# facebookresearch/seamless_communication

Measured on AMD Instinct MI355X. Metric: S2ST utterances/sec (and real-time factor), seamlessM4T_v2_large, 10 s audio, higher is better.
Workload: dtype f32 activations x f16 weights, f32 accumulate

## Files before the change

### seamless_communication_amd/csrc/common.cpp

```cpp
#include "common.h"
#include <cstdlib>
#include <cstring>

namespace sc {

static thread_local char g_err[1024] = "";

void set_error(const char* fmt, ...) {
    va_list ap;
    va_start(ap, fmt);
    vsnprintf(g_err, sizeof(g_err), fmt, ap);
    va_end(ap);
}

const char* get_error() { return g_err; }

namespace knob {
namespace {
struct Knob {
    const char* name;
    int kind;
    const char* what;
};
const Knob knob_table[] = {
    {"SC_DEBUG_NUMERICS", 0, "honour the switches that change results"},
    {"SC_DEBUG_FILL", 0, "fill fresh scratch blocks with NaN (tests)"},
    {"SC_SPLIT_MODE", 1, "1: Conformer products on the hi fp16 plane only (precision study)"},
    {"SC_DECODER_GEN1", 1, "decoder step on the first-generation kernels"},
    {"SC_DECODER_GEN2", 1, "decoder step on the second-generation chain"},
    {"SC_VOC_SPLIT", 1, "vocoder ResBlock products on both fp16 planes of their activations again (bit 0 wide stages, bit 2 narrow stages); default: hi plane only"},
    {"SC_GEMM_GENERAL", 0, "general GEMM kernel instead of the fast path"}, {"SC_GEMM_PF2", 0, "GEMM prefetch depth"},
    {"SC_GEMM_GROUP_M", 0, "GEMM workgroup order"}, {"SC_GEMM_TILE", 0, "GEMM tile override"},
    {"SC_PS_TILE", 0, "DMA GEMM: largest tile"}, {"SC_PS_MIN256", 0, "DMA GEMM: tiles needed for 256 x 256"},
    {"SC_PS_MIN128", 0, "DMA GEMM: tiles needed for 128 x 128"},
    {"SC_PRESPLIT", 0, "0: Conformer operands split on the fly"}, {"SC_ENC_FUSE", 0, "0: separate Conformer element-wise launches"},
    {"SC_D3_RG_SMALL", 0, "decoder step: rows per row group, N = 1024 products"}, {"SC_D3_RG_FFN", 0, "decoder step: rows per row group, FFN-in"},
    {"SC_G3_STATIONARY", 0, "row-group products of wide steps: 0 one workgroup per row group, n = workgroup budget of the weight-stationary launch"},
    {"SC_G3_TILES", 0, "0: FFN-out of wide steps on the weight-stationary row-group walk instead of tile-owning waves"},
    {"SC_G3_TOUCH", 0, "weight-stationary products: bit 0 cooperative L2 touch of the activations, bit 1 K slices per XCD (FFN-out); default 3"},
    {"SC_D3_FFN_IN", 0, "decoder step: FFN-in workgroup shape"}, {"SC_D3_FFN_OUT", 0, "decoder step: FFN-out workgroup shape"},
    {"SC_T2U_GROUPS", 0, "NAR T2U: length buckets"}, {"SC_T2U_PACKED", 0, "0: NAR decoder on padded buckets"},
    {"SC_VOC_PS", 0, "0: vocoder wide stages on the register-staged convolution"}, {"SC_VOC_MRF", 0, "0: narrow vocoder stages as nine pair launches"},
    {"SC_VOC_GROUPS", 0, "vocoder: length buckets"}, {"SC_VOC_GROUP_OVERHEAD", 0, "vocoder: bucket planning overhead rows"},
    {"SC_VOC_STREAMS", 0, "vocoder: side chains"},
    {"SC_VOC_PACKED", 0, "0: ragged vocoder batches in length buckets on side chains instead of the packed pass"},
    {"SC_VOC_PACK_ROWS", 0, "vocoder: unit rows per packed group"},
    {"SC_ENGINE_RG_SMALL", 0, "decode engine: rows per row group, N = 1024 products"},
    {"SC_BEAM_COMPACT", 2, "0: beam search keeps finished utterances' slots"},
    {"SC_GREEDY_COMPACT", 2, "0: greedy generation keeps finished rows in their slots"}, {"SC_GREEDY_POLL", 2, "steps between looks at the finished flags"},
    {"SC_T2U_ENC_PACKED", 2, "0: T2U encoder over the padded rows on the fp32-operand GEMM"},
    {"SC_ENC_GLU_EPI", 2, "0: Conformer conv module writes both GLU halves and gates them in the depthwise kernel"},
};
constexpr int N_KNOBS = sizeof(knob_table) / sizeof(knob_table[0]);
struct State {
    bool set[N_KNOBS];
    int val[N_KNOBS];
    bool numerics = false;
};
const State& state() {
    static const State st = [] {
        State s{};
        const char* dn = getenv("SC_DEBUG_NUMERICS");
        s.numerics = dn && atoi(dn) != 0;
        for (int i = 0; i < N_KNOBS; ++i) {
            const char* e = getenv(knob_table[i].name);
            s.set[i] = e != nullptr && (knob_table[i].kind != 1 || s.numerics);
            s.val[i] = e ? atoi(e) : 0;
        }
        return s;
    }();
    return st;
}
int lookup(const char* name) {
    for (int i = 0; i < N_KNOBS; ++i)
        if (strcmp(knob_table[i].name, name) == 0) return i;
    return -1;
}
int find(const char* name) {
    const int i = lookup(name);
    if (i >= 0) return i;
    fprintf(stderr, "libseamless_hip: switch %s is not in the knob table (common.cpp)\n", name);
    abort();
}
}

bool known(const char* name) { return name && lookup(name) >= 0; }

int value(const char* name, int dflt) {
    const int i = find(name);
    return state().set[i] ? state().val[i] : dflt;
}
bool is_set(const char* name) { return state().set[find(name)]; }
int live(const char* name, int dflt) {
    (void)find(name);
    const char* e = getenv(name);
    return e ? atoi(e) : dflt;
}
void report_once() {
    static const bool done = [] {
        const State& s = state();
        for (int i = 0; i < N_KNOBS; ++i) {
            const char* e = getenv(knob_table[i].name);
            if (!e || knob_table[i].kind == 2) continue;
            if (knob_table[i].kind == 1 && !s.numerics)
                fprintf(stderr, "libseamless_hip: %s=%s IGNORED - it changes results (%s); set SC_DEBUG_NUMERICS=1 to honour it\n", knob_table[i].name, e,
                        knob_table[i].what);
            else
                fprintf(stderr, "libseamless_hip: %s=%s (%s)%s\n", knob_table[i].name, e, knob_table[i].what, knob_table[i].kind == 1 ? " - RESULTS CHANGE" : "");
        }
        return true;
    }();
    (void)done;
}
}

}
```

### seamless_communication_amd/csrc/k_norm.hip

```cpp
#include <vector>

#include "device_util.h"

namespace sc {

__device__ __forceinline__ float act_f(float v, int a) {
    if (a == ACT_RELU) return relu_keep_nan(v);
    if (a == ACT_SILU) return v / (1.f + expf(-v));
    if (a == ACT_GELU) return gelu_erf(v);
    return v;
}

template <int MAXV>
__global__ __launch_bounds__(256) void layernorm_kernel(const float* __restrict__ x, int64_t ldx,
                                                        const float* __restrict__ gamma,
                                                        const float* __restrict__ beta,
                                                        float* __restrict__ y, int64_t ldy, int rows,
                                                        int C, int act, const int* __restrict__ lens,
                                                        int t_per_batch, __half* __restrict__ yh = nullptr,
                                                        __half* __restrict__ yl = nullptr, int64_t ldh = 0) {
    const int lane = threadIdx.x & 63;
    const int row = blockIdx.x * 4 + (threadIdx.x >> 6);
    if (row >= rows) return;
    const int nv = C >> 2;
    const float4* xr = reinterpret_cast<const float4*>(x + (int64_t)row * ldx);
    float4* yr = reinterpret_cast<float4*>(y + (int64_t)row * ldy);
    half4_t* yhr = reinterpret_cast<half4_t*>(yh + (yh ? (int64_t)row * ldh : 0));
    half4_t* ylr = reinterpret_cast<half4_t*>(yl + (yl ? (int64_t)row * ldh : 0));
    const bool both = y != nullptr && yh != nullptr;
    bool masked = false;
    if (lens) {
        const int n = row / t_per_batch;
        const int t = row - n * t_per_batch;
        if (t >= lens[n]) {
            for (int i = lane; i < nv; i += 64) {
                if (yh) {
                    yhr[i] = half4_t{0, 0, 0, 0};
                    ylr[i] = half4_t{0, 0, 0, 0};
                } else {
                    yr[i] = make_float4(0.f, 0.f, 0.f, 0.f);
                }
            }
            if (!both) return;
            masked = true;
        }
    }
    float4 v[MAXV];
    float s = 0.f;
#pragma unroll
    for (int i = 0; i < MAXV; ++i) {
        const int idx = lane + 64 * i;
        v[i] = idx < nv ? xr[idx] : make_float4(0.f, 0.f, 0.f, 0.f);
        s += (v[i].x + v[i].y) + (v[i].z + v[i].w);
    }
    const float mean = wave_sum(s) / (float)C;
    float q = 0.f;
#pragma unroll
    for (int i = 0; i < MAXV; ++i) {
        const int idx = lane + 64 * i;
        if (idx < nv) {
            const float a = v[i].x - mean, b = v[i].y - mean, c = v[i].z - mean, d = v[i].w - mean;
            q += (a * a + b * b) + (c * c + d * d);
        }
    }
    const float var = wave_sum(q) / (float)C;
    const float rstd = 1.0f / sqrtf(var + 1e-5f);
    const float4* g4 = reinterpret_cast<const float4*>(gamma);
    const float4* b4 = reinterpret_cast<const float4*>(beta);
#pragma unroll
    for (int i = 0; i < MAXV; ++i) {
        const int idx = lane + 64 * i;
        if (idx < nv) {
            const float4 g = g4[idx], b = b4[idx];
            float4 o;
            o.x = act_f((v[i].x - mean) * rstd * g.x + b.x, act);
            o.y = act_f((v[i].y - mean) * rstd * g.y + b.y, act);
            o.z = act_f((v[i].z - mean) * rstd * g.z + b.z, act);
            o.w = act_f((v[i].w - mean) * rstd * g.w + b.w, act);
            if (yh && !masked) {
                const f32x4_t of = {o.x, o.y, o.z, o.w};
                const half4_t hi = __builtin_convertvector(of, half4_t);
                const f32x4_t back = __builtin_convertvector(hi, f32x4_t);
                yhr[idx] = hi;
                ylr[idx] = __builtin_convertvector(of - back, half4_t);
            }
            if (!yh || both) yr[idx] = o;
        }
    }
}

__global__ __launch_bounds__(256) void layernorm2_kernel(const float* __restrict__ x, int64_t ldx, const float* __restrict__ ga,
                                                         const float* __restrict__ ba, float* __restrict__ y, int64_t ldy,
                                                         const float* __restrict__ gb2, const float* __restrict__ bb2,
                                                         __half* __restrict__ yh, __half* __restrict__ yl, int64_t ldh, int rows, int C) {
    const int lane = threadIdx.x & 63;
    const int row = blockIdx.x * 4 + (threadIdx.x >> 6);
    if (row >= rows) return;
    const int nv = C >> 2;
    const float4* xr = reinterpret_cast<const float4*>(x + (int64_t)row * ldx);
    float4* yr = reinterpret_cast<float4*>(y + (int64_t)row * ldy);
    half4_t* yhr = reinterpret_cast<half4_t*>(yh + (int64_t)row * ldh);
    half4_t* ylr = reinterpret_cast<half4_t*>(yl + (int64_t)row * ldh);
    float4 v[4];
    float s = 0.f;
#pragma unroll
    for (int i = 0; i < 4; ++i) {
        const int idx = lane + 64 * i;
        v[i] = idx < nv ? xr[idx] : make_float4(0.f, 0.f, 0.f, 0.f);
        s += (v[i].x + v[i].y) + (v[i].z + v[i].w);
    }
    float mean = wave_sum(s) / (float)C;
    float q = 0.f;
#pragma unroll
    for (int i = 0; i < 4; ++i) {
        const int idx = lane + 64 * i;
        if (idx < nv) {
            const float a = v[i].x - mean, b = v[i].y - mean, c = v[i].z - mean, d = v[i].w - mean;
            q += (a * a + b * b) + (c * c + d * d);
        }
    }
    float rstd = 1.0f / sqrtf(wave_sum(q) / (float)C + 1e-5f);
    s = 0.f;
#pragma unroll
    for (int i = 0; i < 4; ++i) {
        const int idx = lane + 64 * i;
        if (idx < nv) {
            const float4 g = reinterpret_cast<const float4*>(ga)[idx], b = reinterpret_cast<const float4*>(ba)[idx];
            v[i].x = (v[i].x - mean) * rstd * g.x + b.x;
            v[i].y = (v[i].y - mean) * rstd * g.y + b.y;
            v[i].z = (v[i].z - mean) * rstd * g.z + b.z;
            v[i].w = (v[i].w - mean) * rstd * g.w + b.w;
            yr[idx] = v[i];
        }
        s += (v[i].x + v[i].y) + (v[i].z + v[i].w);
    }
    mean = wave_sum(s) / (float)C;
    q = 0.f;
#pragma unroll
    for (int i = 0; i < 4; ++i) {
        const int idx = lane + 64 * i;
        if (idx < nv) {
            const float a = v[i].x - mean, b = v[i].y - mean, c = v[i].z - mean, d = v[i].w - mean;
            q += (a * a + b * b) + (c * c + d * d);
        }
    }
    rstd = 1.0f / sqrtf(wave_sum(q) / (float)C + 1e-5f);
#pragma unroll
    for (int i = 0; i < 4; ++i) {
        const int idx = lane + 64 * i;
        if (idx < nv) {
            const float4 g = reinterpret_cast<const float4*>(gb2)[idx], b = reinterpret_cast<const float4*>(bb2)[idx];
            const f32x4_t of = {(v[i].x - mean) * rstd * g.x + b.x, (v[i].y - mean) * rstd * g.y + b.y, (v[i].z - mean) * rstd * g.z + b.z,
                             (v[i].w - mean) * rstd * g.w + b.w};
            const half4_t hi = __builtin_convertvector(of, half4_t);
            const f32x4_t back = __builtin_convertvector(hi, f32x4_t);
            yhr[idx] = hi;
            ylr[idx] = __builtin_convertvector(of - back, half4_t);
        }
    }
}

void launch_layernorm2_split(const float* x, int64_t ldx, const float* ga, const float* ba, float* y, int64_t ldy, const float* gb2,
                             const float* bb2, __half* yh, __half* yl, int64_t ldh, int rows, int C, hipStream_t s) {
    SC_CHECK(C % 4 == 0 && C <= 1024 && ldx % 4 == 0 && ldy % 4 == 0 && ldh % 4 == 0 && y && yh && yl, "layernorm2_split: C=%d", C);
    if (rows <= 0) return;
    hipLaunchKernelGGL(layernorm2_kernel, dim3(cdiv(rows, 4)), dim3(256), 0, s, x, ldx, ga, ba, y, ldy, gb2, bb2, yh, yl, ldh, rows, C);
    SC_LAUNCH_CHECK();
}

void launch_layernorm_split(const float* x, int64_t ldx, const float* gamma, const float* beta, __half* yh, __half* yl,
                            int64_t ldh, int rows, int C, int act, const int* lens, int t_per_batch, hipStream_t s) {
    SC_CHECK(C % 4 == 0 && ldx % 4 == 0 && ldh % 4 == 0 && C <= 4096 && yh && yl, "layernorm_split: C=%d ldx=%lld ldh=%lld", C,
             (long long)ldx, (long long)ldh);
    if (rows <= 0) return;
    dim3 grid(cdiv(rows, 4));
    float* none = nullptr;
    if (C <= 256) hipLaunchKernelGGL((layernorm_kernel<1>), grid, dim3(256), 0, s, x, ldx, gamma, beta, none, (int64_t)0, rows, C, act, lens, t_per_batch, yh, yl, ldh);
    else if (C <= 1024) hipLaunchKernelGGL((layernorm_kernel<4>), grid, dim3(256), 0, s, x, ldx, gamma, beta, none, (int64_t)0, rows, C, act, lens, t_per_batch, yh, yl, ldh);
    else hipLaunchKernelGGL((layernorm_kernel<16>), grid, dim3(256), 0, s, x, ldx, gamma, beta, none, (int64_t)0, rows, C, act, lens, t_per_batch, yh, yl, ldh);
    SC_LAUNCH_CHECK();
}

void launch_layernorm_both(const float* x, int64_t ldx, const float* gamma, const float* beta, float* y, int64_t ldy, __half* yh,
                           __half* yl, int64_t ldh, int rows, int C, int act, const int* lens, int t_per_batch, hipStream_t s) {
    SC_CHECK(C % 4 == 0 && ldx % 4 == 0 && ldy % 4 == 0 && ldh % 4 == 0 && C <= 4096 && y && yh && yl, "layernorm_both: C=%d", C);
    if (rows <= 0) return;
    dim3 grid(cdiv(rows, 4));
    if (C <= 256) hipLaunchKernelGGL((layernorm_kernel<1>), grid, dim3(256), 0, s, x, ldx, gamma, beta, y, ldy, rows, C, act, lens, t_per_batch, yh, yl, ldh);
    else if (C <= 1024) hipLaunchKernelGGL((layernorm_kernel<4>), grid, dim3(256), 0, s, x, ldx, gamma, beta, y, ldy, rows, C, act, lens, t_per_batch, yh, yl, ldh);
    else hipLaunchKernelGGL((layernorm_kernel<16>), grid, dim3(256), 0, s, x, ldx, gamma, beta, y, ldy, rows, C, act, lens, t_per_batch, yh, yl, ldh);
    SC_LAUNCH_CHECK();
}

void launch_layernorm(const float* x, int64_t ldx, const float* gamma, const float* beta, float* y,
                      int64_t ldy, int rows, int C, int act, const int* lens, int t_per_batch,
                      hipStream_t s) {
    SC_CHECK(C % 4 == 0 && ldx % 4 == 0 && ldy % 4 == 0, "layernorm: C=%d ldx=%lld ldy=%lld must be multiples of 4", C,
             (long long)ldx, (long long)ldy);
    SC_CHECK(C <= 4096, "layernorm: C=%d > 4096 unsupported", C);
    if (rows <= 0) return;
    dim3 grid(cdiv(rows, 4));
    if (C <= 256) {
        hipLaunchKernelGGL((layernorm_kernel<1>), grid, dim3(256), 0, s, x, ldx, gamma, beta, y, ldy, rows, C, act, lens, t_per_batch, (__half*)nullptr, (__half*)nullptr, (int64_t)0);
    } else if (C <= 1024) {
        hipLaunchKernelGGL((layernorm_kernel<4>), grid, dim3(256), 0, s, x, ldx, gamma, beta, y, ldy, rows, C, act, lens, t_per_batch, (__half*)nullptr, (__half*)nullptr, (int64_t)0);
    } else {
        hipLaunchKernelGGL((layernorm_kernel<16>), grid, dim3(256), 0, s, x, ldx, gamma, beta, y, ldy, rows, C, act, lens, t_per_batch, (__half*)nullptr, (__half*)nullptr, (int64_t)0);
    }
    SC_LAUNCH_CHECK();
}

__global__ __launch_bounds__(256) void glu_kernel(const float* __restrict__ x, int64_t ldx,
                                                  float* __restrict__ y, int64_t ldy, int rows, int C) {
    const int cv = C >> 2;
    const int64_t total = (int64_t)rows * cv;
    for (int64_t i = (int64_t)blockIdx.x * blockDim.x + threadIdx.x; i < total;
         i += (int64_t)gridDim.x * blockDim.x) {
        const int r = (int)(i / cv);
        const int c = (int)(i - (int64_t)r * cv);
        const float4 a = *reinterpret_cast<const float4*>(x + (int64_t)r * ldx + c * 4);
        const float4 g = *reinterpret_cast<const float4*>(x + (int64_t)r * ldx + C + c * 4);
        float4 o;
        o.x = a.x / (1.f + expf(-g.x));
        o.y = a.y / (1.f + expf(-g.y));
        o.z = a.z / (1.f + expf(-g.z));
        o.w = a.w / (1.f + expf(-g.w));
        *reinterpret_cast<float4*>(y + (int64_t)r * ldy + c * 4) = o;
    }
}

void launch_glu(const float* x, int64_t ldx, float* y, int64_t ldy, int rows, int C, hipStream_t s) {
    SC_CHECK(C % 4 == 0 && ldx % 4 == 0 && ldy % 4 == 0, "glu: alignment");
    if (rows <= 0) return;
    const int64_t total = (int64_t)rows * (C / 4);
    const int blocks = (int)std::min<int64_t>(cdiv64(total, 256), 4096);
    hipLaunchKernelGGL(glu_kernel, dim3(blocks), dim3(256), 0, s, x, ldx, y, ldy, rows, C);
    SC_LAUNCH_CHECK();
}

template <int K, int TT>
__global__ __launch_bounds__(256) void glu_dwconv_kernel(const float* __restrict__ x, int64_t ldx,
                                                         const float* __restrict__ w,
                                                         float* __restrict__ y, int64_t ldy, int T,
                                                         int C, const int* __restrict__ lens, int left,
                                                         const float* __restrict__ bn_scale,
                                                         const float* __restrict__ bn_shift) {
    const int c = blockIdx.x * 256 + threadIdx.x;
    const int t0 = blockIdx.y * TT;
    const int n = blockIdx.z;
    if (c >= C) return;
    const int len = lens ? min(lens[n], T) : T;
    float wr[K];
#pragma unroll
    for (int j = 0; j < K; ++j) wr[j] = w[c * K + j];
    float g[TT + K - 1];
#pragma unroll
    for (int i = 0; i < TT + K - 1; ++i) {
        const int t = t0 - left + i;
        float v = 0.f;
        if (t >= 0 && t < len) {
            const float* xr = x + ((int64_t)n * T + t) * ldx;
            const float a = xr[c];
            const float b = xr[C + c];
            v = a / (1.f + expf(-b));
        }
        g[i] = v;
    }
#pragma unroll
    for (int tt = 0; tt < TT; ++tt) {
        const int t = t0 + tt;
        if (t < T) {
            float acc = 0.f;
#pragma unroll
            for (int j = 0; j < K; ++j) acc = fmaf(wr[j], g[tt + j], acc);
            if (bn_scale) {
                acc = fmaf(acc, bn_scale[c], bn_shift[c]);
                acc = acc / (1.f + expf(-acc));
            }
            y[((int64_t)n * T + t) * ldy + c] = acc;
        }
    }
}

__global__ __launch_bounds__(256) void glu_dwconv_generic_kernel(const float* __restrict__ x, int64_t ldx,
                                                                 const float* __restrict__ w,
                                                                 float* __restrict__ y, int64_t ldy,
                                                                 int T, int C, int K,
                                                                 const int* __restrict__ lens, int left,
                                                                 const float* __restrict__ bn_scale,
                                                                 const float* __restrict__ bn_shift) {
    const int c = blockIdx.x * 256 + threadIdx.x;
    const int t = blockIdx.y;
    const int n = blockIdx.z;
    if (c >= C) return;
    const int len = lens ? min(lens[n], T) : T;
    float acc = 0.f;
    for (int j = 0; j < K; ++j) {
        const int ts = t - left + j;
        if (ts >= 0 && ts < len) {
            const float* xr = x + ((int64_t)n * T + ts) * ldx;
            acc = fmaf(w[c * K + j], xr[c] / (1.f + expf(-xr[C + c])), acc);
        }
    }
    if (bn_scale) {
        acc = fmaf(acc, bn_scale[c], bn_shift[c]);
        acc = acc / (1.f + expf(-acc));
    }
    y[((int64_t)n * T + t) * ldy + c] = acc;
}

__global__ void bn_fold_kernel(const float* __restrict__ g, const float* __restrict__ b, const float* __restrict__ mean,
                               const float* __restrict__ var, float eps, int C, float* __restrict__ scale, float* __restrict__ shift) {
    const int c = blockIdx.x * blockDim.x + threadIdx.x;
    if (c >= C) return;
    const float sc = g[c] / sqrtf(var[c] + eps);
    scale[c] = sc;
    shift[c] = b[c] - mean[c] * sc;
}

void launch_bn_fold(const float* g, const float* b, const float* mean, const float* var, float eps, int C, float* scale, float* shift,
                    hipStream_t s) {
    hipLaunchKernelGGL(bn_fold_kernel, dim3(cdiv(C, 256)), dim3(256), 0, s, g, b, mean, var, eps, C, scale, shift);
    SC_LAUNCH_CHECK();
}

__global__ void relpos_table_kernel(int S, int M, float* __restrict__ out) {
    const int idx = blockIdx.x * blockDim.x + threadIdx.x;
    const int half = M / 2;
    if (idx >= (2 * S - 1) * half) return;
    const int t = idx / half, i = idx - t * half;
    const float pos = (float)((S - 1) - t);
    const float div = expf((float)(2 * i) * -(logf(10000.0f) / (float)M));
    const float a = pos * div;
    out[(int64_t)t * M + 2 * i] = sinf(a);
    out[(int64_t)t * M + 2 * i + 1] = cosf(a);
}

void launch_relpos_table(int S, int M, float* out, hipStream_t s) {
    hipLaunchKernelGGL(relpos_table_kernel, dim3(cdiv((2 * S - 1) * (M / 2), 256)), dim3(256), 0, s, S, M, out);
    SC_LAUNCH_CHECK();
}

template <int K, int TT, bool GATED, bool PACKED = false>
__global__ __launch_bounds__(1024) void glu_dwconv_ln_kernel(const float* __restrict__ x, int64_t ldx, const float* __restrict__ w,
                                                             const float* __restrict__ gamma, const float* __restrict__ beta, int act,
                                                             __half* __restrict__ yh, __half* __restrict__ yl, int64_t ldh, int T, int C,
                                                             const int* __restrict__ lens, int range) {
    __shared__ float tile[2][TT][1024];
    const int c = threadIdx.x;
    const int lane = c & 63, wv = c >> 6, waves = C >> 6;
    int4 wk = {0, 0, 0, 0};
    if constexpr (PACKED) wk = reinterpret_cast<const int4*>(lens)[blockIdx.x];
    const int n = blockIdx.y;
    const int t_begin = PACKED ? wk.z : blockIdx.x * range, t_end = PACKED ? min(wk.w, wk.y) : min(T, t_begin + range);
    if (t_begin >= t_end) return;
    const int len = PACKED ? wk.y : (lens ? min(lens[n], T) : T);
    const float* xn = PACKED ? x + (int64_t)wk.x * ldx : x + (int64_t)n * T * ldx;
    float wr[K];
#pragma unroll
    for (int j = 0; j < K; ++j) wr[j] = w[c * K + j];
    float g[TT + K - 1];
#pragma unroll
    for (int i = 0; i < K - 1; ++i) {
        const int t = t_begin - (K - 1) + i;
        float v = 0.f;
        if (t >= 0 && t < len) {
            const float a = xn[(int64_t)t * ldx + c];
            if constexpr (GATED) {
                v = a;
            } else {
                const float b = xn[(int64_t)t * ldx + C + c];
                v = a / (1.f + expf(-b));
            }
        }
        g[i] = v;
    }
    float ra[TT], rb[TT];
    (void)rb;
#pragma unroll
    for (int i = 0; i < TT; ++i) {
        const int t = t_begin + i;
        const bool ok = t < t_end && t < len;
        ra[i] = ok ? xn[(int64_t)t * ldx + c] : 0.f;
        if constexpr (!GATED) rb[i] = ok ? xn[(int64_t)t * ldx + C + c] : 0.f;
    }
    const int nv = C >> 2;
    int buf = 0;
    for (int tc = t_begin; tc < t_end; tc += TT) {
#pragma unroll
        for (int i = 0; i < TT; ++i) {
            const int t = tc + i;
            if constexpr (GATED) g[K - 1 + i] = (t < t_end && t < len) ? ra[i] : 0.f;
            else g[K - 1 + i] = (t < t_end && t < len) ? ra[i] / (1.f + expf(-rb[i])) : 0.f;
        }
#pragma unroll
        for (int i = 0; i < TT; ++i) {
            const int t = tc + TT + i;
            const bool ok = t < t_end && t < len;
            ra[i] = ok ? xn[(int64_t)t * ldx + c] : 0.f;
            if constexpr (!GATED) rb[i] = ok ? xn[(int64_t)t * ldx + C + c] : 0.f;
        }
#pragma unroll
        for (int tt = 0; tt < TT; ++tt) {
            float acc = 0.f;
#pragma unroll
            for (int j = 0; j < K; ++j) acc = fmaf(wr[j], g[tt + j], acc);
            tile[buf][tt][c] = acc;
        }
        __syncthreads();
        for (int r = wv; r < TT && tc + r < t_end; r += waves) {
            const float4* xr = reinterpret_cast<const float4*>(&tile[buf][r][0]);
            const int64_t row = PACKED ? (int64_t)wk.x + tc + r : (int64_t)n * T + tc + r;
            half4_t* yhr = reinterpret_cast<half4_t*>(yh + row * ldh);
            half4_t* ylr = reinterpret_cast<half4_t*>(yl + row * ldh);
            float s = 0.f;
#pragma unroll
            for (int i = 0; i < 4; ++i) {
                const int idx = lane + 64 * i;
                const float4 vv = idx < nv ? xr[idx] : make_float4(0.f, 0.f, 0.f, 0.f);
                s += (vv.x + vv.y) + (vv.z + vv.w);
            }
            const float mean = wave_sum(s) / (float)C;
            float q = 0.f;
#pragma unroll
            for (int i = 0; i < 4; ++i) {
                const int idx = lane + 64 * i;
                if (idx < nv) {
                    const float4 vv = xr[idx];
                    const float a = vv.x - mean, b = vv.y - mean, cc = vv.z - mean, d = vv.w - mean;
                    q += (a * a + b * b) + (cc * cc + d * d);
                }
            }
            const float var = wave_sum(q) / (float)C;
            const float rstd = 1.0f / sqrtf(var + 1e-5f);
            const float4* g4 = reinterpret_cast<const float4*>(gamma);
            const float4* b4 = reinterpret_cast<const float4*>(beta);
#pragma unroll
            for (int i = 0; i < 4; ++i) {
                const int idx = lane + 64 * i;
                if (idx < nv) {
                    const float4 gg = g4[idx], bb = b4[idx], vv = xr[idx];
                    float4 o;
                    o.x = act_f((vv.x - mean) * rstd * gg.x + bb.x, act);
                    o.y = act_f((vv.y - mean) * rstd * gg.y + bb.y, act);
                    o.z = act_f((vv.z - mean) * rstd * gg.z + bb.z, act);
                    o.w = act_f((vv.w - mean) * rstd * gg.w + bb.w, act);
                    const f32x4_t of = {o.x, o.y, o.z, o.w};
                    const half4_t hi = __builtin_convertvector(of, half4_t);
                    const f32x4_t back = __builtin_convertvector(hi, f32x4_t);
                    yhr[idx] = hi;
                    ylr[idx] = __builtin_convertvector(of - back, half4_t);
                }
            }
        }
#pragma unroll
        for (int i = 0; i < K - 1; ++i) g[i] = g[i + TT];
        buf ^= 1;
    }
}

bool glu_dwconv_ln_supported(int C, int ksize) { return ksize == 31 && C % 64 == 0 && C >= 64 && C <= 1024; }

void launch_glu_dwconv_ln(const float* x, int64_t ldx, const float* w, const float* gamma, const float* beta, int act, __half* yh,
                          __half* yl, int64_t ldh, int nb, int T, int C, int ksize, const int* lens, hipStream_t s, bool gated) {
    SC_CHECK(glu_dwconv_ln_supported(C, ksize) && ldh % 4 == 0, "glu_dwconv_ln: C=%d k=%d ldh=%lld unsupported", C, ksize, (long long)ldh);
    if (nb <= 0 || T <= 0) return;
    constexpr int TT = 8;
    int ranges = std::max(1, std::min(cdiv(256, nb), cdiv(T, 32)));
    const int range = cdiv(cdiv(T, ranges), TT) * TT;
    ranges = cdiv(T, range);
    const double rows = (double)nb * T;
    prof::Scope scope("glu_dwconv_ln", 2.0 * rows * C * ksize, rows * C * ((gated ? 4.0 : 8.0) + 4.0), s);
    if (gated)
        hipLaunchKernelGGL((glu_dwconv_ln_kernel<31, TT, true>), dim3(ranges, nb), dim3(C), 0, s, x, ldx, w, gamma, beta, act, yh, yl, ldh, T, C,
                           lens, range);
    else
        hipLaunchKernelGGL((glu_dwconv_ln_kernel<31, TT, false>), dim3(ranges, nb), dim3(C), 0, s, x, ldx, w, gamma, beta, act, yh, yl, ldh, T, C,
                           lens, range);
    SC_LAUNCH_CHECK();
}

void glu_dwconv_ln_packed_work(const int32_t* row_off, const int32_t* lens, int n, std::vector<int32_t>& work) {
    constexpr int TT = 8;
    work.clear();
    int64_t R = 0;
    for (int i = 0; i < n; ++i) R += std::max(lens[i], 0);
    const int per_wg = (int)std::max<int64_t>(32, cdiv64(cdiv64(R, 256), TT) * TT);
    for (int i = 0; i < n; ++i) {
        const int len = lens[i];
        if (len <= 0) continue;
        const int ranges = std::max(1, std::min(cdiv(len, per_wg), cdiv(len, 32)));
        const int range = cdiv(cdiv(len, ranges), TT) * TT;
        for (int t = 0; t < len; t += range) {
            const int32_t rec[4] = {row_off[i], len, t, std::min(len, t + range)};
            work.insert(work.end(), rec, rec + 4);
        }
    }
}

void launch_glu_dwconv_ln_packed(const float* x, int64_t ldx, const float* w, const float* gamma, const float* beta, int act, __half* yh,
                                 __half* yl, int64_t ldh, const int* d_work, int n_work, double rows, int C, int ksize, hipStream_t s,
                                 bool gated) {
    SC_CHECK(glu_dwconv_ln_supported(C, ksize) && ldh % 4 == 0 && (reinterpret_cast<uintptr_t>(d_work) & 15) == 0,
             "glu_dwconv_ln_packed: C=%d k=%d ldh=%lld unsupported", C, ksize, (long long)ldh);
    if (n_work <= 0) return;
    constexpr int TT = 8;
    prof::Scope scope("glu_dwconv_ln_packed", 2.0 * rows * C * ksize, rows * C * ((gated ? 4.0 : 8.0) + 4.0), s);
    if (gated)
        hipLaunchKernelGGL((glu_dwconv_ln_kernel<31, TT, true, true>), dim3(n_work), dim3(C), 0, s, x, ldx, w, gamma, beta, act, yh, yl, ldh, 0, C,
                           d_work, 0);
    else
        hipLaunchKernelGGL((glu_dwconv_ln_kernel<31, TT, false, true>), dim3(n_work), dim3(C), 0, s, x, ldx, w, gamma, beta, act, yh, yl, ldh, 0, C,
                           d_work, 0);
    SC_LAUNCH_CHECK();
}

void launch_glu_dwconv(const float* x, int64_t ldx, const float* w, float* y, int64_t ldy, int nb, int T,
                       int C, int ksize, const int* lens, hipStream_t s, int left, const float* bn_scale, const float* bn_shift) {
    if (nb <= 0 || T <= 0) return;
    if (left < 0) left = ksize - 1;
    if (ksize == 31) {
        constexpr int TT = 16;
        dim3 grid(cdiv(C, 256), cdiv(T, TT), nb);
        hipLaunchKernelGGL((glu_dwconv_kernel<31, TT>), grid, dim3(256), 0, s, x, ldx, w, y, ldy, T, C, lens, left, bn_scale, bn_shift);
    } else {
        dim3 grid(cdiv(C, 256), T, nb);
        hipLaunchKernelGGL(glu_dwconv_generic_kernel, grid, dim3(256), 0, s, x, ldx, w, y, ldy, T, C, ksize, lens, left, bn_scale, bn_shift);
    }
    SC_LAUNCH_CHECK();
}

}
```

Before: 339.6.

## Rewrite Conformer glu_dwconv_ln with register sliding window and multi-channel threads

Adds a new glu_dwconv_ln kernel that keeps the 31-tap depthwise window and the weights in registers. In the gated path each thread handles two channels over a 16-step tile. It prefetches the next tile's inputs while the current tile is convolved, and double-buffers convolution outputs in dynamic LDS, where each wave runs a LayerNorm row pass with a fp16 hi/lo split. The previous one-channel-per-thread kernel stays as a fallback, chosen by the SC_GDL_V1 switch or when the input is misaligned. The aim is to cut repeated loads of the input window and improve latency hiding, at the cost of higher register pressure and fewer threads per block.

```diff
diff --git a/seamless_communication_amd/csrc/common.cpp b/seamless_communication_amd/csrc/common.cpp
--- a/seamless_communication_amd/csrc/common.cpp
+++ b/seamless_communication_amd/csrc/common.cpp
@@ -50,6 +50,7 @@
     {"SC_GREEDY_COMPACT", 2, "0: greedy generation keeps finished rows in their slots"}, {"SC_GREEDY_POLL", 2, "steps between looks at the finished flags"},
     {"SC_T2U_ENC_PACKED", 2, "0: T2U encoder over the padded rows on the fp32-operand GEMM"},
     {"SC_ENC_GLU_EPI", 2, "0: Conformer conv module writes both GLU halves and gates them in the depthwise kernel"},
+    {"SC_GDL_V1", 2, "1: Conformer conv module middle (glu_dwconv_ln) on the one-channel-per-thread kernel"},
 };
 constexpr int N_KNOBS = sizeof(knob_table) / sizeof(knob_table[0]);
 struct State {
diff --git a/seamless_communication_amd/csrc/k_norm.hip b/seamless_communication_amd/csrc/k_norm.hip
--- a/seamless_communication_amd/csrc/k_norm.hip
+++ b/seamless_communication_amd/csrc/k_norm.hip
@@ -342,10 +342,10 @@
 }
 
 template <int K, int TT, bool GATED, bool PACKED = false>
-__global__ __launch_bounds__(1024) void glu_dwconv_ln_kernel(const float* __restrict__ x, int64_t ldx, const float* __restrict__ w,
-                                                             const float* __restrict__ gamma, const float* __restrict__ beta, int act,
-                                                             __half* __restrict__ yh, __half* __restrict__ yl, int64_t ldh, int T, int C,
-                                                             const int* __restrict__ lens, int range) {
+__global__ __launch_bounds__(1024) void glu_dwconv_ln_v1_kernel(const float* __restrict__ x, int64_t ldx, const float* __restrict__ w,
+                                                                const float* __restrict__ gamma, const float* __restrict__ beta, int act,
+                                                                __half* __restrict__ yh, __half* __restrict__ yl, int64_t ldh, int T, int C,
+                                                                const int* __restrict__ lens, int range) {
     __shared__ float tile[2][TT][1024];
     const int c = threadIdx.x;
     const int lane = c & 63, wv = c >> 6, waves = C >> 6;
@@ -459,7 +459,190 @@
     }
 }
 
+template <int ACT>
+__device__ __forceinline__ void gdl_norm_row(const float4* xr, const float4* g4, const float4* b4, int act, half4_t* yhr, half4_t* ylr, int lane,
+                                             int nv, int C) {
+    const int a_ = ACT >= 0 ? ACT : act;
+    float s = 0.f;
+#pragma unroll
+    for (int i = 0; i < 4; ++i) {
+        const int idx = lane + 64 * i;
+        const float4 vv = idx < nv ? xr[idx] : make_float4(0.f, 0.f, 0.f, 0.f);
+        s += (vv.x + vv.y) + (vv.z + vv.w);
+    }
+    const float mean = wave_sum(s) / (float)C;
+    float q = 0.f;
+#pragma unroll
+    for (int i = 0; i < 4; ++i) {
+        const int idx = lane + 64 * i;
+        if (idx < nv) {
+            const float4 vv = xr[idx];
+            const float a = vv.x - mean, b = vv.y - mean, cc = vv.z - mean, d = vv.w - mean;
+            q += (a * a + b * b) + (cc * cc + d * d);
+        }
+    }
+    const float var = wave_sum(q) / (float)C;
+    const float rstd = 1.0f / sqrtf(var + 1e-5f);
+#pragma unroll
+    for (int i = 0; i < 4; ++i) {
+        const int idx = lane + 64 * i;
+        const int idc = min(idx, nv - 1);
+        const float4 gg = g4[idc], bb = b4[idc], vv = xr[idc];
+        float4 o;
+        o.x = act_f((vv.x - mean) * rstd * gg.x + bb.x, a_);
+        o.y = act_f((vv.y - mean) * rstd * gg.y + bb.y, a_);
+        o.z = act_f((vv.z - mean) * rstd * gg.z + bb.z, a_);
+        o.w = act_f((vv.w - mean) * rstd * gg.w + bb.w, a_);
+        const f32x4_t of = {o.x, o.y, o.z, o.w};
+        const half4_t hi = __builtin_convertvector(of, half4_t);
+        const f32x4_t back = __builtin_convertvector(hi, f32x4_t);
+        if (idx < nv) {
+            yhr[idx] = hi;
+            ylr[idx] = __builtin_convertvector(of - back, half4_t);
+        }
+    }
+}
+
+template <int K, int TT, bool GATED, bool PACKED, int CH>
+__global__ __launch_bounds__(1024 / CH) void glu_dwconv_ln_kernel(const float* __restrict__ x, int64_t ldx, const float* __restrict__ w,
+                                                                  const float* __restrict__ gamma, const float* __restrict__ beta, int act,
+                                                                  __half* __restrict__ yh, __half* __restrict__ yl, int64_t ldh, int T, int C,
+                                                                  const int* __restrict__ lens, int range) {
+    typedef float vec_t __attribute__((ext_vector_type(CH)));
+    extern __shared__ __attribute__((aligned(16))) float tile_dyn[];
+    const int lane = threadIdx.x & 63, wv = threadIdx.x >> 6, waves = blockDim.x >> 6;
+    const bool live = CH * (int)threadIdx.x < C;
+    const int c = live ? CH * (int)threadIdx.x : 0;
+    int4 wk = {0, 0, 0, 0};
+    if constexpr (PACKED) wk = reinterpret_cast<const int4*>(lens)[blockIdx.x];
+    const int n = blockIdx.y;
+    const int t_begin = PACKED ? wk.z : blockIdx.x * range, t_end = PACKED ? min(wk.w, wk.y) : min(T, t_begin + range);
+    if (t_begin >= t_end) return;
+    const int len = PACKED ? wk.y : (lens ? min(lens[n], T) : T);
+    const float* xn = (PACKED ? x + (int64_t)wk.x * ldx : x + (int64_t)n * T * ldx) + c;
+    vec_t zero;
+#pragma unroll
+    for (int e = 0; e < CH; ++e) zero[e] = 0.f;
+    auto load = [&](int t, int off) { return *reinterpret_cast<const vec_t*>(xn + (int64_t)t * ldx + off); };
+    auto glu = [&](vec_t a, vec_t b) {
+        if constexpr (!GATED) {
+#pragma unroll
+            for (int e = 0; e < CH; ++e) a[e] = a[e] / (1.f + expf(-b[e]));
+        }
+        return a;
+    };
+    vec_t wr[K];
+#pragma unroll
+    for (int j = 0; j < K; ++j)
+#pragma unroll
+        for (int e = 0; e < CH; ++e) wr[j][e] = w[(c + e) * K + j];
+    vec_t g[TT + K - 1];
+#pragma unroll
+    for (int i = 0; i < K - 1; ++i) {
+        const int t = t_begin - (K - 1) + i;
+        vec_t v = zero;
+        if (live && t >= 0 && t < len) {
+            vec_t b = zero;
+            if constexpr (!GATED) b = load(t, C);
+            v = glu(load(t, 0), b);
+        }
+        g[i] = v;
+    }
+    vec_t ra[TT], rb[GATED ? 1 : TT];
+    (void)rb;
+#pragma unroll
+    for (int i = 0; i < TT; ++i) {
+        const int t = t_begin + i;
+        const bool ok = live && t < t_end && t < len;
+        ra[i] = ok ? load(t, 0) : zero;
+        if constexpr (!GATED) rb[i] = ok ? load(t, C) : zero;
+    }
+    const int nv = C >> 2;
+    float* lds_g = tile_dyn + 2 * TT * C;
+    for (int i = threadIdx.x; i < C; i += blockDim.x) {
+        lds_g[i] = gamma[i];
+        lds_g[C + i] = beta[i];
+    }
+    const float4* g4 = reinterpret_cast<const float4*>(lds_g);
+    const float4* b4 = reinterpret_cast<const float4*>(lds_g + C);
+    const int trips = (t_end - t_begin + TT - 1) / TT;
+    for (int k = 0; k <= trips; ++k) {
+        const int tc = t_begin + k * TT;
+        float* tile = tile_dyn + (k & 1) * TT * C;
+#pragma unroll
+        for (int i = 0; i < TT; ++i) {
+            const int t = tc + i;
+            vec_t v = zero;
+            if constexpr (GATED) v = ra[i];
+            else if (t < t_end && t < len) v = glu(ra[i], rb[i]);
+            g[K - 1 + i] = v;
+        }
+        if (k > 0) {
+            const float* prev = tile_dyn + ((k - 1) & 1) * TT * C;
+            for (int r = wv; r < TT && tc - TT + r < t_end; r += waves) {
+                const float4* xr = reinterpret_cast<const float4*>(prev + r * C);
+                const int64_t row = (PACKED ? (int64_t)wk.x : (int64_t)n * T) + tc - TT + r;
+                half4_t* yhr = reinterpret_cast<half4_t*>(yh + row * ldh);
+                half4_t* ylr = reinterpret_cast<half4_t*>(yl + row * ldh);
+                if (act == ACT_SILU) gdl_norm_row<ACT_SILU>(xr, g4, b4, act, yhr, ylr, lane, nv, C);
+                else if (act == ACT_NONE) gdl_norm_row<ACT_NONE>(xr, g4, b4, act, yhr, ylr, lane, nv, C);
+                else gdl_norm_row<-1>(xr, g4, b4, act, yhr, ylr, lane, nv, C);
+            }
+        }
+        if (k == trips) break;
+#pragma unroll
+        for (int i = 0; i < TT; ++i) {
+            const int t = tc + TT + i;
+            const bool ok = live && t < t_end && t < len;
+            ra[i] = ok ? load(t, 0) : zero;
+            if constexpr (!GATED) rb[i] = ok ? load(t, C) : zero;
+        }
+        if (live) {
+#pragma unroll
+            for (int tt = 0; tt < TT; tt += 4) {
+                vec_t acc[4] = {zero, zero, zero, zero};
+#pragma unroll
+                for (int j = 0; j < K; ++j)
+#pragma unroll
+                    for (int u = 0; u < 4; ++u) acc[u] = __builtin_elementwise_fma(wr[j], g[tt + u + j], acc[u]);
+#pragma unroll
+                for (int u = 0; u < 4; ++u) *reinterpret_cast<vec_t*>(tile + (tt + u) * C + c) = acc[u];
+            }
+        }
+#pragma unroll
+        for (int i = 0; i < K - 1; ++i) g[i] = g[i + TT];
+        __syncthreads();
+    }
+}
+
 bool glu_dwconv_ln_supported(int C, int ksize) { return ksize == 31 && C % 64 == 0 && C >= 64 && C <= 1024; }
+
+static int gdl_variant(const float* x, int64_t ldx) {
+    if (knob::live("SC_GDL_V1", 0) != 0) return 1;
+    return (ldx % 2 == 0 && (reinterpret_cast<uintptr_t>(x) & 7) == 0) ? 0 : 1;
+}
+
+template <bool GATED, bool PACKED, int CH, int TT>
+static void gdl_launch_cfg(dim3 grid, hipStream_t s, const float* x, int64_t ldx, const float* w, const float* gamma, const float* beta, int act,
+                           __half* yh, __half* yl, int64_t ldh, int T, int C, const int* lens, int range) {
+    static bool attr_set = false;
+    if (!attr_set) {
+        SC_HIP(hipFuncSetAttribute(reinterpret_cast<const void*>(&glu_dwconv_ln_kernel<31, TT, GATED, PACKED, CH>),
+                                   hipFuncAttributeMaxDynamicSharedMemorySize, (2 * TT + 2) * 1024 * (int)sizeof(float)));
+        attr_set = true;
+    }
+    const int threads = cdiv(C / CH, 64) * 64;
+    const size_t lds = (size_t)(2 * TT + 2) * C * sizeof(float);
+    hipLaunchKernelGGL((glu_dwconv_ln_kernel<31, TT, GATED, PACKED, CH>), grid, dim3(threads), lds, s, x, ldx, w, gamma, beta, act, yh, yl, ldh,
+                       T, C, lens, range);
+}
+
+template <bool GATED, bool PACKED>
+static void gdl_launch(dim3 grid, hipStream_t s, const float* x, int64_t ldx, const float* w, const float* gamma, const float* beta,
+                       int act, __half* yh, __half* yl, int64_t ldh, int T, int C, const int* lens, int range) {
+    if constexpr (GATED) gdl_launch_cfg<GATED, PACKED, 2, 16>(grid, s, x, ldx, w, gamma, beta, act, yh, yl, ldh, T, C, lens, range);
+    else gdl_launch_cfg<GATED, PACKED, 1, 8>(grid, s, x, ldx, w, gamma, beta, act, yh, yl, ldh, T, C, lens, range);
+}
 
 void launch_glu_dwconv_ln(const float* x, int64_t ldx, const float* w, const float* gamma, const float* beta, int act, __half* yh,
                           __half* yl, int64_t ldh, int nb, int T, int C, int ksize, const int* lens, hipStream_t s, bool gated) {
@@ -471,11 +654,15 @@
     ranges = cdiv(T, range);
     const double rows = (double)nb * T;
     prof::Scope scope("glu_dwconv_ln", 2.0 * rows * C * ksize, rows * C * ((gated ? 4.0 : 8.0) + 4.0), s);
-    if (gated)
-        hipLaunchKernelGGL((glu_dwconv_ln_kernel<31, TT, true>), dim3(ranges, nb), dim3(C), 0, s, x, ldx, w, gamma, beta, act, yh, yl, ldh, T, C,
+    const int variant = gdl_variant(x, ldx);
+    if (variant != 1) {
+        if (gated) gdl_launch<true, false>(dim3(ranges, nb), s, x, ldx, w, gamma, beta, act, yh, yl, ldh, T, C, lens, range);
+        else gdl_launch<false, false>(dim3(ranges, nb), s, x, ldx, w, gamma, beta, act, yh, yl, ldh, T, C, lens, range);
+    } else if (gated)
+        hipLaunchKernelGGL((glu_dwconv_ln_v1_kernel<31, TT, true>), dim3(ranges, nb), dim3(C), 0, s, x, ldx, w, gamma, beta, act, yh, yl, ldh, T, C,
                            lens, range);
     else
-        hipLaunchKernelGGL((glu_dwconv_ln_kernel<31, TT, false>), dim3(ranges, nb), dim3(C), 0, s, x, ldx, w, gamma, beta, act, yh, yl, ldh, T, C,
+        hipLaunchKernelGGL((glu_dwconv_ln_v1_kernel<31, TT, false>), dim3(ranges, nb), dim3(C), 0, s, x, ldx, w, gamma, beta, act, yh, yl, ldh, T, C,
                            lens, range);
     SC_LAUNCH_CHECK();
 }
@@ -506,11 +693,15 @@
     if (n_work <= 0) return;
     constexpr int TT = 8;
     prof::Scope scope("glu_dwconv_ln_packed", 2.0 * rows * C * ksize, rows * C * ((gated ? 4.0 : 8.0) + 4.0), s);
-    if (gated)
-        hipLaunchKernelGGL((glu_dwconv_ln_kernel<31, TT, true, true>), dim3(n_work), dim3(C), 0, s, x, ldx, w, gamma, beta, act, yh, yl, ldh, 0, C,
+    const int variant = gdl_variant(x, ldx);
+    if (variant != 1) {
+        if (gated) gdl_launch<true, true>(dim3(n_work), s, x, ldx, w, gamma, beta, act, yh, yl, ldh, 0, C, d_work, 0);
+        else gdl_launch<false, true>(dim3(n_work), s, x, ldx, w, gamma, beta, act, yh, yl, ldh, 0, C, d_work, 0);
+    } else if (gated)
+        hipLaunchKernelGGL((glu_dwconv_ln_v1_kernel<31, TT, true, true>), dim3(n_work), dim3(C), 0, s, x, ldx, w, gamma, beta, act, yh, yl, ldh, 0, C,
                            d_work, 0);
     else
-        hipLaunchKernelGGL((glu_dwconv_ln_kernel<31, TT, false, true>), dim3(n_work), dim3(C), 0, s, x, ldx, w, gamma, beta, act, yh, yl, ldh, 0, C,
+        hipLaunchKernelGGL((glu_dwconv_ln_v1_kernel<31, TT, false, true>), dim3(n_work), dim3(C), 0, s, x, ldx, w, gamma, beta, act, yh, yl, ldh, 0, C,
                            d_work, 0);
     SC_LAUNCH_CHECK();
 }
```

After: 340.5 (median of 6 runs). No clear change (+0.3%).
